# B-R-P/NMSLIB-ZIG

Measured on AMD Instinct MI355X. Metric: queries/sec @ recall@10, 1M x 128-D L2, batch=1024; HBM GB/s vs peak, higher is better.
Workload: dtype f16+f32

## Files before the change

nmslib_zig_amd/csrc/kernels/bf_kernels.hip:

```cpp
#include <cstdio>
#include <type_traits>
#include <vector>
#include <cstdlib>

#include "common_dev.hpp"
#include "kernels.hpp"

namespace gfxknn {

enum BfMode : int { BF_L2 = 0, BF_DOT = 1, BF_COS = 2, BF_L1 = 3, BF_LINF = 4, BF_COSC = 5, BF_L2D = 6 };

struct BfArgs {
    const float* base;
    const float* aux;
    const float* qaux;
    int aux_stride;
    const float* queries;
    u64* cand;
    int* cand_cnt;
    uint32_t* gthr;
    uint32_t* gq;
    int xj, xm;
    int n, ldb, nqt, nsplit, rows_per_split, kprime, cap;
    int kcs;
// ... 1893 lines not shown

__device__ __forceinline__ float one_product_error(const float* qs, int dim, int lane, float bscale, float bres, float scale) {
    float ss = 0.f, rr = 0.f;
    bool over = false;
    for (int d = lane; d < dim; d += 64) {
        const float v = scale * qs[d], w = v - (float)(_Float16)v;
        over |= !(fabsf(v) <= 65504.f);
        ss = fmaf(v, v, ss);
        rr = fmaf(w, w, rr);
    }
    const float qn = sqrtf(wave_sum(ss)), qr = sqrtf(wave_sum(rr));
    if (__any(over)) return INFINITY;
    return 1.01f * (qr * bscale + 1.004f * qn * bres) + 2e-5f * qn * bscale;
}

template <int NPER>
__global__ __launch_bounds__(256) void bf_f32_threshold_kernel(const float* top8, int nlists, int depth, int r, int rcap, int nq,
                                                               int qpad, const float* queries_sel, int ldb, int dim, float bscale,
                                                               float bres, int group_q, int force_precise, float* thr3,
                                                               float* thr1, int* precise, float scale_q, float unit) {
    const int lane = threadIdx.x & 63, q = blockIdx.x * 4 + (threadIdx.x >> 6);
    if (q >= qpad) return;
    if (q >= nq) {
        if (lane == 0) {
            thr3[q] = INFINITY;
            thr1[q] = INFINITY;
        }
        return;
    }
    const int total = nlists * depth;
    uint32_t key[NPER];
#pragma unroll
    for (int i = 0; i < NPER; ++i) {
        const int idx = i * 64 + lane;
        const int l = depth == 4 ? idx >> 2 : idx >> 3, j = idx - l * depth;
        key[i] = idx < total ? f32_ord(top8[((size_t)q * nlists + l) * 8 + j]) : 0u;
    }
    const float e1 = one_product_error(queries_sel + (size_t)q * ldb, dim, lane, bscale, bres, scale_q);
    const uint32_t T = total >= r ? wave_rth_largest_u32<NPER>(key, r) : 0u;
    const float t3 = total >= r ? ord_f32(T) : -INFINITY;
    float t1 = t3;
    bool ok = force_precise != 1;
    if (ok && t3 > -INFINITY) {
        const float need = 2.1f * e1;
        uint32_t best = 0u;
#pragma unroll
        for (int i = 0; i < NPER; ++i) {
            const float v = ord_f32(key[i]);
            const bool c = key[i] != 0u && key[i] <= T && v > -INFINITY && t3 - v >= need;
            best = c && key[i] > best ? key[i] : best;
        }
#pragma unroll
        for (int o = 32; o > 0; o >>= 1) {
// ... 4 lines not shown
        if (best != 0u) {
            int above = 0;
#pragma unroll
            for (int i = 0; i < NPER; ++i) above += __popcll(__builtin_amdgcn_ballot_w64(key[i] > best));
            const int jmax = rcap < total ? rcap : total;
            const int j = best == T ? r : above + 1;
            if (j <= jmax) {
                t1 = ord_f32(best);
                ok = true;
            }
        }
    }
    if (lane == 0) {
        thr3[q] = (t3 - 1.02f * e1) / unit;
        thr1[q] = force_precise == 2 ? INFINITY : t1;
        if (!ok) atomicOr(&precise[q / group_q], 1);
    }
}

struct RerankListF32Args {
    const float* base;
    const float* queries;
    const uint32_t* list;
    const int* list_cnt;
    const int32_t* ext_ids;
    int32_t* out_ids;
    float* out_dists;
    int32_t* out_cnt;
    int* tile_fail;
    int n, k, nsplit, caph, p2max, fail_queries, space, dim, ldb;
    int tps;
    const float* queries_sel;
    const float* thr;
    const float* thr1;
    const int* precise;
    int no_split;
    float bmax;
    float bres;
    float scale, scale_q, bres16;
    int sel_dim, sel_ld;
    const float* qaux;
    unsigned long long* prof;
};

__global__ __launch_bounds__(256) void bf_rerank_f32_list_kernel(RerankListF32Args a) {
    const unsigned long long t0 = a.prof ? wall_clock64() : 0;
    auto lap = [&](int i) __attribute__((always_inline)) {
        if (a.prof && threadIdx.x == 0) atomicAdd(&a.prof[i], wall_clock64() - t0);
    };
    extern __shared__ __attribute__((aligned(16))) char smem[];
    u64* keys = reinterpret_cast<u64*>(smem);
    int* offs = reinterpret_cast<int*>(keys + a.p2max);
    __shared__ int s_over, s_split;
    __shared__ float s_qn2, s_e1, s_thr;
    const int q = blockIdx.x, tid = threadIdx.x, lane = tid & 63, wave = tid >> 6;
    const int nl = 2 * a.nsplit;
    if (tid == 0) s_over = 0;
    __syncthreads();
    if (tid < 64) {
        const int per = (nl + 63) / 64;
        int sum = 0, over = 0;
        for (int i = 0; i < per; ++i) {
            const int s = tid * per + i;
            if (s < nl) {
                const int c = a.list_cnt[(size_t)q * nl + s];
                over |= c > a.caph;
                sum += c < a.caph ? c : a.caph;
            }
        }
        int incl = sum;
#pragma unroll
        for (int o = 1; o < 64; o <<= 1) {
            const int v = __shfl_up(incl, o, 64);
            if (tid >= o) incl += v;
        }
        int run = incl - sum;
        for (int i = 0; i < per; ++i) {
            const int s = tid * per + i;
            if (s < nl) {
                offs[s] = run;
                const int c = a.list_cnt[(size_t)q * nl + s];
                run += c < a.caph ? c : a.caph;
            }
        }
        if (tid == 63) offs[nl] = incl;
        if (__any(over != 0) && tid == 0) s_over = 1;
    } else if (wave == 1) {
        const bool split_product = a.precise[q / a.fail_queries] != 0;
        const float* qs = a.queries_sel + (size_t)q * a.sel_ld;
        float ss = 0.f;
        for (int d = lane; d < a.sel_dim; d += 64) ss = fmaf(qs[d], qs[d], ss);
        ss = wave_sum(ss);
        const float e1 = split_product ? 0.f : one_product_error(qs, a.sel_dim, lane, a.scale * (a.space == SP_L2 || a.space == SP_NEGDOT || a.qaux ? a.bmax : 1.0f), a.bres16, a.scale_q);
        if (lane == 0) {
            s_qn2 = ss;
            s_e1 = e1;
            s_split = split_product ? 1 : 0;
            s_thr = split_product ? a.thr[q] : a.thr1[q];
        }
    }
    __syncthreads();
    const int total = offs[nl];
    if ((a.no_split && a.precise[q / a.fail_queries] != 0) ||
        (a.qaux && a.qaux[(size_t)q * 4 + 3] == 0.f)) {
        if (tid == 0) atomicOr(&a.tile_fail[q / a.fail_queries], 1);
        return;
    }
    const int need = a.k < a.n ? a.k : a.n;
    const int want = need + (a.k / 8 > 4 ? a.k / 8 : 4) < a.n ? need + (a.k / 8 > 4 ? a.k / 8 : 4) : a.n;
    if (s_over || total < want || total > a.p2max) {
        if (tid == 0) atomicOr(&a.tile_fail[q / a.fail_queries], 1);
        return;
    }
    lap(0);
    scan_gather_entries(keys, offs, a.list, q, nl, a.caph, a.tps, tid, blockDim.x);
    __syncthreads();
    lap(1);
    const int P = next_pow2(total < 2 ? 2 : total);
    if (a.prof && tid == 0) {
        atomicAdd(&a.prof[8], (unsigned long long)total);
        atomicAdd(&a.prof[9], (unsigned long long)P);
        atomicAdd(&a.prof[10], 1ull);
    }
    const float* qq = a.queries + (size_t)q * a.ldb;
    const int sub = lane & 15, rg = lane >> 4;
    if (a.dim <= 128) {
        float qv[8];
        bool ok[8];
    #pragma unroll
        for (int c = 0; c < 8; ++c) {
            const int d = sub + 16 * c;
            ok[c] = d < a.dim;
            qv[c] = ok[c] ? qq[d] : 0.f;
        }
        constexpr int kU = 4;
        for (int j0 = wave * (4 * kU); j0 < total; j0 += 16 * kU) {
            uint32_t pos[kU];
            float xv[kU][8];
    #pragma unroll
            for (int u = 0; u < kU; ++u) {
                const int j = j0 + 4 * u + rg;
                pos[u] = (uint32_t)keys[j < total ? j : total - 1];
                const float* row = a.base + (size_t)pos[u] * a.ldb + sub;
    #pragma unroll
                for (int c = 0; c < 8; ++c) xv[u][c] = ok[c] ? row[16 * c] : 0.f;
            }
            __builtin_amdgcn_wave_barrier();
    #pragma unroll
            for (int u = 0; u < kU; ++u) {
                float p0[4], p1[4], p2[4];
    #pragma unroll
                for (int v = 0; v < 4; ++v) {
                    p0[v] = p1[v] = p2[v] = 0.f;
    #pragma unroll
                    for (int c = 0; c < 2; ++c) {
                        if (64 * c >= a.dim) continue;
                        const float x = xv[u][v + 4 * c], y = qv[v + 4 * c];
                        if (a.space == SP_L2) {
                            const float t = x - y;
                            p0[v] = fmaf(t, t, p0[v]);
                        } else {
                            p0[v] = fmaf(x, y, p0[v]);
                            if (a.space != SP_NEGDOT) {
                                p1[v] = fmaf(x, x, p1[v]);
                                p2[v] = fmaf(y, y, p2[v]);
                            }
                        }
                    }
                }
                auto tree = [&](const float* p) __attribute__((always_inline)) -> float {
                    float s = (p[0] + p[2]) + (p[1] + p[3]);
    #pragma unroll
                    for (int o = 8; o > 0; o >>= 1) s += __shfl_xor(s, o, 64);
                    return s;
                };
                const float s0 = tree(p0);
                float d;
                if (a.space == SP_L2) d = sqrtf(s0);
                else if (a.space == SP_NEGDOT) d = -s0;
                else {
                    const float sim = normdot_finish(s0, tree(p1), tree(p2));
                    d = a.space == SP_ANGULAR ? acosf(sim) : fmaxf(0.0f, 1.0f - sim);
                }
                const int j = j0 + 4 * u + rg;
                if (sub == 0 && j < total) keys[j] = ((u64)f32_ord(d) << 32) | pos[u];
            }
        }
    } else {
        const int nstep = (a.dim + 63) >> 6;
        for (int j0 = wave * 16; j0 < total; j0 += 64) {
            uint32_t pos[4];
            const float* rowp[4];
    #pragma unroll
            for (int u = 0; u < 4; ++u) {
                const int j = j0 + 4 * u + rg;
                pos[u] = (uint32_t)keys[j < total ? j : total - 1];
                rowp[u] = a.base + (size_t)pos[u] * a.ldb + sub;
            }
            float p0[4][4], p1[4][4], p2[4][4];
    #pragma unroll
            for (int u = 0; u < 4; ++u)
    #pragma unroll
                for (int v = 0; v < 4; ++v) p0[u][v] = p1[u][v] = p2[u][v] = 0.f;
            for (int c0 = 0; c0 < nstep; c0 += 2) {
                float xv[4][8], qv[8];
                bool ok[8];
    #pragma unroll
                for (int c = 0; c < 8; ++c) {
                    const int d = sub + 16 * (c & 3) + 64 * (c0 + (c >> 2));
                    ok[c] = d < a.dim;
                    qv[c] = ok[c] ? qq[d] : 0.f;
    #pragma unroll
                    for (int u = 0; u < 4; ++u) xv[u][c] = ok[c] ? rowp[u][16 * (c & 3) + 64 * (c0 + (c >> 2))] : 0.f;
                }
    #pragma unroll
                for (int u = 0; u < 4; ++u) {
    #pragma unroll
                    for (int v = 0; v < 4; ++v) {
    #pragma unroll
                        for (int c = 0; c < 2; ++c) {
                            if (64 * (c0 + c) >= a.dim) continue;
                            const float x = xv[u][v + 4 * c], y = qv[v + 4 * c];
                            if (a.space == SP_L2) {
                                const float t = x - y;
                                p0[u][v] = fmaf(t, t, p0[u][v]);
                            } else {
                                p0[u][v] = fmaf(x, y, p0[u][v]);
                                if (a.space != SP_NEGDOT) {
                                    p1[u][v] = fmaf(x, x, p1[u][v]);
                                    p2[u][v] = fmaf(y, y, p2[u][v]);
                                }
                            }
                        }
                    }
                }
            }
            __builtin_amdgcn_wave_barrier();
    #pragma unroll
            for (int u = 0; u < 4; ++u) {
                auto tree = [&](const float* p) __attribute__((always_inline)) -> float {
                    float s = (p[0] + p[2]) + (p[1] + p[3]);
    #pragma unroll
                    for (int o = 8; o > 0; o >>= 1) s += __shfl_xor(s, o, 64);
                    return s;
                };
                const float s0 = tree(p0[u]);
                float d;
                if (a.space == SP_L2) d = sqrtf(s0);
                else if (a.space == SP_NEGDOT) d = -s0;
                else {
                    const float sim = normdot_finish(s0, tree(p1[u]), tree(p2[u]));
                    d = a.space == SP_ANGULAR ? acosf(sim) : fmaxf(0.0f, 1.0f - sim);
                }
                const int j = j0 + 4 * u + rg;
                if (sub == 0 && j < total) keys[j] = ((u64)f32_ord(d) << 32) | pos[u];
            }
        }
    }
    __syncthreads();
    lap(2);
    if (total <= 512 && a.k <= 32) {
        __shared__ u64 s_head[128];
        const int e0 = wave * 128 + 2 * lane;
        u64 k0 = e0 < total ? keys[e0] : ~0ull, k1 = e0 + 1 < total ? keys[e0 + 1] : ~0ull;
        wave_sort128_u64(k0, k1, lane);
        if (lane < 16) {
            s_head[wave * 32 + 2 * lane] = k0;
            s_head[wave * 32 + 2 * lane + 1] = k1;
        }
        __syncthreads();
        if (wave == 0) {
            k0 = s_head[2 * lane];
            k1 = s_head[2 * lane + 1];
            wave_sort128_u64(k0, k1, lane);
            if (lane < 16) {
                keys[2 * lane] = k0;
                keys[2 * lane + 1] = k1;
            }
        }
        __syncthreads();
    } else {
        for (int i = total + tid; i < P; i += blockDim.x) keys[i] = ~0ull;
        __syncthreads();
        block_bitonic_u64_asc(keys, P, tid, blockDim.x);
    }
    lap(3);
    const int found = total < a.k ? total : a.k;
    if (total < a.n) {
        const bool split_product = s_split != 0;
        if (tid == 0) {
            const float qn2 = s_qn2, qn = sqrtf(qn2);
            const float dk = ord_f32((uint32_t)(keys[found - 1] >> 32));
            float sk, e, extra = 0.f;
            if (a.qaux) {
                const float sh = sinf(0.5f * dk);
                const float omc = a.space == SP_ANGULAR ? 2.0f * sh * sh : dk;
                const float qnorm = a.qaux[(size_t)q * 4 + 2];
                sk = -omc * qnorm;
                e = 6.1036e-5f * qn * a.bmax;
                extra = 1e-6f * qn * a.bmax + 2e-6f * qnorm;
            } else if (a.space == SP_L2) {
                sk = 0.5f * (qn2 - dk * dk);
                e = 6.1036e-5f * qn * a.bmax;
            } else if (a.space == SP_NEGDOT) {
                sk = -dk;
                e = 6.1036e-5f * qn * a.bmax;
            } else {
                sk = (a.space == SP_ANGULAR ? cosf(dk) : 1.0f - dk) * qn;
                e = 6.1036e-5f * qn;
            }
            const float t = s_thr;
            if (!split_product) {
                const float unit = a.scale * a.scale_q;
                sk *= unit;
                extra *= unit;
                e = s_e1;
            }
            e += extra + 1e-6f * (fabsf(sk) + fabsf(t));
            if (!(sk - t >= e)) atomicOr(&a.tile_fail[q / a.fail_queries], 1);
        }
    }
    lap(4);
    for (int i = tid; i < a.k; i += blockDim.x) {
        int32_t id = -1;
        float d = INFINITY;
        if (i < found) {
            const u64 key = keys[i];
            const uint32_t pos = (uint32_t)key;
            id = a.ext_ids ? a.ext_ids[pos] : (int32_t)pos;
            d = ord_f32((uint32_t)(key >> 32));
        }
        a.out_ids[(size_t)q * a.k + i] = id;
        a.out_dists[(size_t)q * a.k + i] = d;
    }
    if (tid == 0 && a.out_cnt) a.out_cnt[q] = found;
    lap(5);
}

__global__ void row_maxnorm_kernel(const float* rows, int n, int ld, int dim, int relative, unsigned* out_bits, float scale16) {
    const int lane = threadIdx.x & 63;
    const int wpb = blockDim.x >> 6;
    float mb = 0.f, mr = 0.f, ma = 0.f, mh = 0.f;
    for (int row = blockIdx.x * wpb + (threadIdx.x >> 6); row < n; row += gridDim.x * wpb) {
        const float* p = rows + (size_t)row * ld;
        float s = 0.f, r = 0.f, rh = 0.f;
        for (int d = lane; d < dim; d += 64) {
            const float v = p[d], w = v - (float)(__bf16)v;
            const float vs = scale16 * v, wh = vs - (float)(_Float16)vs;
            s = fmaf(v, v, s);
            r = fmaf(w, w, r);
            rh = fmaf(wh, wh, rh);
// ... 21 lines not shown
    const void* queries;
    const u64* cand;
    const int* cand_cnt;
    const int32_t* ext_ids;
    int32_t* out_ids;
    float* out_dists;
    int32_t* out_cnt;
    int space, dim, ldb, k, nsplit, cap, kprime, p2max;
    const int* tile_fail;
    int fail_queries;
    int* verify_flags;
    int verify_queries;
    const float* queries_sel;
    float bmax;
    float eps_rel;
};

__global__ __launch_bounds__(256) void bf_rerank_kernel(RerankArgs a) {
    extern __shared__ __attribute__((aligned(16))) char smem[];
    u64* keys = reinterpret_cast<u64*>(smem);
    int* offs = reinterpret_cast<int*>(keys + a.p2max);
    const int q = blockIdx.x, tid = threadIdx.x, lane = tid & 63, wave = tid >> 6;
    if (a.tile_fail && a.tile_fail[q / a.fail_queries] == 0) return;

    if (tid == 0) {
        int o = 0;
        for (int s = 0; s < a.nsplit; ++s) {
            offs[s] = o;
            int c = a.cand_cnt[(size_t)q * a.nsplit + s];
            o += c < a.kprime ? c : a.kprime;
        }
        offs[a.nsplit] = o;
    }
    __syncthreads();
    const int total = offs[a.nsplit];
    __shared__ uint32_t s_kth;
    const bool verify = a.verify_flags != nullptr && a.space == SP_L2 && total >= a.kprime;
    if (tid == 0) s_kth = 0xffffffffu;
// ... 76 lines not shown
            const float* qs = a.queries_sel + (size_t)q * a.ldb;
            float ss = 0.f;
            for (int d = tid; d < a.dim; d += 64) ss = fmaf(qs[d], qs[d], ss);
            ss = wave_sum(ss);
            if (tid == 0) s_qn2v = ss;
        }
        __syncthreads();
        if (tid == 0) {
            const float qn2 = s_qn2v, qn = sqrtf(qn2);
            const float kth = ord_f32(s_kth);
            const float dk = ord_f32((uint32_t)(keys[found - 1] >> 32));
            const float e = a.eps_rel * (qn * a.bmax + 0.5f * a.bmax * a.bmax);
            const float floor_d2 = qn2 - 2.0f * kth - 2.0f * e - 2e-6f * (qn2 + fabsf(kth));
            if (!(dk * dk <= floor_d2)) atomicOr(&a.verify_flags[q / a.verify_queries], 1);
        }
    }
}

__global__ void row_aux_f32_kernel(const float* base, int n, int ldb, int dim, int space, float* aux) {
    const int lane = threadIdx.x & 63;
    const int row = blockIdx.x * (blockDim.x >> 6) + (threadIdx.x >> 6);
    if (row >= n) return;
    const float* p = base + (size_t)row * ldb;
    float s = 0.f;
    for (int d = lane; d < dim; d += 64) s = fmaf(p[d], p[d], s);
    s = wave_sum(s);
    if (lane == 0) {
        float v = 0.f;
        if (space == SP_L2) v = -0.5f * s;
        else if (space == SP_COSINE || space == SP_ANGULAR)
// ... 522 lines not shown
                            const int* cand_cnt, const int32_t* ext_ids, int32_t* out_ids,
                            float* out_dists, int32_t* out_cnt, hipStream_t s) {
    return launch_bf_rerank_ex(p, space, dim, k, base, queries_padded, cand, cand_cnt, ext_ids, out_ids, out_dists,
                               out_cnt, nullptr, 1, s);
}

hipError_t launch_bf_rerank_ex(const BfPlan& p, int space, int dim, int k, const void* base,
                               const void* queries_padded, const unsigned long long* cand,
                               const int* cand_cnt, const int32_t* ext_ids, int32_t* out_ids,
                               float* out_dists, int32_t* out_cnt, const int* tile_fail, int fail_queries,
                               hipStream_t s) {
    return launch_bf_rerank_verify(p, space, dim, k, base, queries_padded, cand, cand_cnt, ext_ids, out_ids, out_dists,
                                   out_cnt, tile_fail, fail_queries, nullptr, nullptr, 0.f, s);
}

hipError_t launch_bf_rerank_verify(const BfPlan& p, int space, int dim, int k, const void* base,
                                   const void* queries_padded, const unsigned long long* cand,
                                   const int* cand_cnt, const int32_t* ext_ids, int32_t* out_ids,
                                   float* out_dists, int32_t* out_cnt, const int* tile_fail, int fail_queries,
                                   int* verify_flags, const float* queries_sel, float bmax, hipStream_t s) {
    RerankArgs a{};
    a.verify_flags = verify_flags;
    a.verify_queries = BF_TQ;
    a.queries_sel = queries_sel;
    a.bmax = bmax;
    a.eps_rel = 1.5f * (float)(dim + 2) * 5.9604645e-8f;
    a.tile_fail = tile_fail;
    a.fail_queries = fail_queries;
    a.base = base;
    a.queries = queries_padded;
// ... 2 lines not shown
    a.ext_ids = ext_ids;
    a.out_ids = out_ids;
    a.out_dists = out_dists;
    a.out_cnt = out_cnt;
    a.space = space;
    a.dim = dim;
    a.ldb = p.ldb;
    a.k = k;
    a.nsplit = p.nsplit;
    a.cap = p.cap;
    a.kprime = p.kprime;
    a.p2max = p.p2max;
    hipError_t e = hipFuncSetAttribute(reinterpret_cast<const void*>(bf_rerank_kernel),
                                       hipFuncAttributeMaxDynamicSharedMemorySize, (int)p.lds_rerank);
    if (e != hipSuccess) return e;
    hipLaunchKernelGGL(bf_rerank_kernel, dim3(p.nq), dim3(256), p.lds_rerank, s, a);
    return hipGetLastError();
}

hipError_t launch_bf_adaptive_f32(const BfPlan& p, int space, int dim, int k, const float* base_orig, const float* sel_rows,
                                  const float* aux, const float* queries_orig, const float* queries_sel,
                                  const float* qaux_cosc, float bmax, unsigned long long* cand, int* cand_cnt, int* flags,
                                  const int32_t* ext_ids, int32_t* out_ids, float* out_dists, int32_t* out_cnt,
                                  const int* gate, int gate_tiles, hipStream_t s, bool cleared) {
    hipError_t e = launch_bf_select_f32_ex(p, space, sel_rows, aux, queries_sel, qaux_cosc, cand, cand_cnt, gate, gate_tiles, s,
                                           cleared);
    if (e != hipSuccess) return e;
    const bool verify = space == SP_L2 && flags != nullptr && bmax > 0.f;
    if (!verify)
        return launch_bf_rerank_ex(p, space, dim, k, base_orig, queries_orig, cand, cand_cnt, ext_ids, out_ids, out_dists,
                                   out_cnt, gate, gate_tiles * BF_TQ, s);
// ... 180 lines not shown
    if (const char* e = getenv("NMSLIB_GPU_SAMPLE_STRIDE")) f.stride = atoi(e) > 0 ? atoi(e) : 16;
    const int kp = k + (k / 8 > 4 ? k / 8 : 4);
    const double kf = (double)kp / f.stride;
    f.r = (int)(1.6 * kf + 3.0 * sqrt(kf) + 3.0 + 0.999);
    f.rcap = 4 * f.r + 32;
    f.force_precise = false;
    if (const char* e = getenv("NMSLIB_GPU_F32_TERMS")) f.force_precise = atoi(e) == 3;
    const int tiles_all = (n + BF_BN - 1) / BF_BN;
    int ns = (256 + f.nqt - 1) / f.nqt;
    if (ns > tiles_all / 16) ns = tiles_all / 16;
    if (ns > 256) ns = 256;
    ns = (ns + 7) / 8 * 8;
    if (ns < 8) ns = 8;
    while ((tiles_all + ns - 1) / ns > 32768) ns += 8;
    f.nsplit = ns;
    f.tps = (tiles_all + ns - 1) / ns;
    const double mean_half = (double)f.rcap * f.stride / (2.0 * ns);
    int caph = 8;
    while (caph < 3.0 * mean_half + 8.0) caph <<= 1;
    f.caph = caph;
    f.p2max = host_next_pow2((int)(2.5 * f.rcap * f.stride) + 64);
    if (f.p2max > 2 * ns * caph) f.p2max = host_next_pow2(2 * ns * caph);
    f.lds_scan = 4 * 2 * BF_BN * 256 + 8 * BF_BN * 4 + 64;
    f.lds_scan1 = 9 * BF_BN * 256 + 16 * BF_BN * 4 + 64;
    f.lds_rerank = (size_t)f.p2max * 8 + (2 * (size_t)ns + 1) * 4 + 16;
    const int stiles = (tiles_all + f.stride - 1) / f.stride;
    const int s_nqt = f.qpad / (f.kch > 1 ? 128 : 256);
    int nss = (256 + s_nqt - 1) / s_nqt;
    if (nss > stiles / 16) nss = stiles / 16;
    if (nss > 64) nss = 64;
// ... 76 lines not shown
    if (qg == 2) return launch_scan_f32_one<MODE, false, 4>(a, grid, lds, s);
    return launch_scan_f32_one<MODE, false, 2>(a, grid, lds, s);
}

hipError_t launch_bf_f32_fast(const BfF32Fast& f, int space, int n, int dim, int ldb, int nq, int k, const float* base_orig,
                              const float* sel_rows, const float* aux, const void* base_hi, const void* base_lo,
                              const float* auxp, float bmax, float bres, const float* queries_orig, const float* queries_sel,
                              void* q_hi, void* q_lo, float* top8, unsigned long long* cand_fb, int* cnt_fb, float* thr,
                              uint32_t* list, int* list_cnt, int* tile_fail, int* flags_fb, const int32_t* ext_ids,
                              int32_t* out_ids, float* out_dists, int32_t* out_cnt, hipEvent_t scan_begin,
                              hipEvent_t scan_end, hipStream_t s, const float* queries_raw, float* queries_pad_out,
                              const float* qaux_cosc, const float* queries_centred, int sel_ld, const BfF16Side& h16) {
    const int sdim = f.cosc ? f.sel_dim : dim, sld = f.cosc ? sel_ld : ldb;
    float* thr1 = thr + f.qpad;
    int* precise = tile_fail + f.nqt;
    hipError_t e;
    {
        const BfPlan& fb = f.fallback;
        uint32_t* gthr = reinterpret_cast<uint32_t*>(cnt_fb + (size_t)fb.qpad * fb.nsplit);
        const size_t gwords = 2 * ((size_t)fb.qpad + (size_t)fb.qpad * fb.nsplit);
        size_t work = (size_t)f.qpad * f.dp > gwords ? (size_t)f.qpad * f.dp : gwords;
        size_t grid = (work + 255) / 256;
        if (grid > 2048) grid = 2048;
        hipLaunchKernelGGL(bf_f32_prep_kernel, dim3((unsigned)grid), dim3(256), 0, s, queries_raw, nq, sdim, queries_sel, f.qpad,
                           sld, queries_pad_out, f.kch > 1 ? nullptr : static_cast<__bf16*>(q_hi),
                           f.kch > 1 ? nullptr : static_cast<__bf16*>(q_lo),
                           tile_fail, 2 * f.nqt, flags_fb, fb.nqt, gthr, gwords, f.dp, static_cast<_Float16*>(h16.q_h16), h16.scale_q);
        e = hipGetLastError();
        if (e != hipSuccess) return e;
    }
// ... 20 lines not shown
    a.nqt = f.nqt;
    BfScanF32Args sa = a;
    sa.nqt = f.qpad / (f.kch > 1 ? 128 : 256);
    sa.nsplit = f.s_nsplit;
    sa.tps = f.s_tps;
    sa.tile_stride = f.stride;
    sa.top8 = top8;
    e = scan(sa, true, 1, 8 * sa.nqt * (f.s_nsplit / 8));
    if (e != hipSuccess) return e;
    {
        static const bool dbg_nohit = getenv("NMSLIB_GPU_DEBUG") && (atoi(getenv("NMSLIB_GPU_DEBUG")) & 8192);
        const int depth = f.rcap <= 64 && f.s_nsplit >= 32 ? 4 : 8;
        const dim3 tgrid((f.qpad + 3) / 4);
#define BF_THR_ARGS                                                                                                               \
    top8, 2 * f.s_nsplit, depth, f.r, f.rcap, nq, f.qpad, queries_sel, sld, sdim, h16.scale * (f.mode == 2 ? 1.0f : bmax), h16.bres16, f.tq, \
        f.force_precise ? 1 : (dbg_nohit ? 2 : 0), thr, thr1, precise, h16.scale_q, h16.scale * h16.scale_q
        if (2 * f.s_nsplit * depth <= 512) hipLaunchKernelGGL(bf_f32_threshold_kernel<8>, tgrid, dim3(256), 0, s, BF_THR_ARGS);
        else hipLaunchKernelGGL(bf_f32_threshold_kernel<16>, tgrid, dim3(256), 0, s, BF_THR_ARGS);
#undef BF_THR_ARGS
    }
    e = hipGetLastError();
    if (e != hipSuccess) return e;
    a.list = list;
    a.list_cnt = list_cnt;
    a.nsplit = f.nsplit;
    a.tps = f.tps;
    a.caph = f.caph;
    a.tile_stride = 1;
    a.group_flag = precise;
    const int grid = 8 * f.nqt * (f.nsplit / 8);
    if (scan_begin) (void)hipEventRecord(scan_begin, s);
// ... 26 lines not shown
    r.p2max = f.p2max;
    r.fail_queries = f.tq;
    r.no_split = f.kch > 1 ? 1 : 0;
    r.space = space;
    r.dim = dim;
    r.ldb = ldb;
    r.queries_sel = queries_sel;
    r.sel_dim = sdim;
    r.sel_ld = sld;
    r.scale = h16.scale;
    r.scale_q = h16.scale_q;
    r.bres16 = h16.bres16;
    r.qaux = f.cosc ? qaux_cosc : nullptr;
    r.thr = thr;
    r.thr1 = thr1;
    r.precise = precise;
    r.bmax = bmax;
    r.bres = bres;
    static const int dbg_prof = getenv("NMSLIB_GPU_DEBUG") ? atoi(getenv("NMSLIB_GPU_DEBUG")) : 0;
    static unsigned long long* d_prof = nullptr;
    if (dbg_prof & 4096) {
        if (!d_prof) (void)hipMalloc(&d_prof, 16 * 8);
        (void)hipMemsetAsync(d_prof, 0, 16 * 8, s);
        r.prof = d_prof;
    }
    e = hipFuncSetAttribute(reinterpret_cast<const void*>(bf_rerank_f32_list_kernel),
                            hipFuncAttributeMaxDynamicSharedMemorySize, (int)f.lds_rerank);
    if (e != hipSuccess) return e;
    hipLaunchKernelGGL(bf_rerank_f32_list_kernel, dim3(nq), dim3(256), f.lds_rerank, s, r);
    e = hipGetLastError();
    if (e != hipSuccess) return e;
    if (dbg_prof & 4096) {
        unsigned long long h[16];
        (void)hipStreamSynchronize(s);
        (void)hipMemcpy(h, d_prof, sizeof(h), hipMemcpyDeviceToHost);
        const double wg = h[10] ? (double)h[10] : 1.0;
        fprintf(stderr, "[rerank f32 list] workgroups %llu rows/query %.1f P %.1f | us since start: prefix %.2f gather %.2f distances %.2f "
                "sort %.2f proof %.2f out %.2f\n", h[10], h[8] / wg, h[9] / wg, h[0] / wg / 100, h[1] / wg / 100, h[2] / wg / 100,
                h[3] / wg / 100, h[4] / wg / 100, h[5] / wg / 100);
    }
    {
        static const int dbg = getenv("NMSLIB_GPU_DEBUG") ? atoi(getenv("NMSLIB_GPU_DEBUG")) : 0;
        if (dbg & 2048) {
            (void)hipStreamSynchronize(s);
// ... 134 lines not shown
```

nmslib_zig_amd/csrc/kernels/kernels.hpp:

```cpp
#pragma once
#include <hip/hip_runtime_api.h>
#include <stddef.h>
#include <stdint.h>

namespace gfxknn {

enum SpaceCode : int {
    SP_L2 = 0,
    SP_L1 = 1,
    SP_LINF = 2,
    SP_COSINE = 3,
    SP_ANGULAR = 4,
    SP_NEGDOT = 5,
    SP_L2SQR_SIFT = 6,
    SP_L2SQR = 7,
    SP_NORMCOS = 8,
    SP_QNORM_NEGDOT = 9,
    SP_LEVEN = 10,
    SP_BIT_HAMMING = 11,
};

constexpr int BF_TQ = 128;
constexpr int BF_BN = 64;
constexpr int BF_KC = 128;
// ... 74 lines not shown
    bool cosc;
    int sel_dim;
    int kch;
    int dp;
    int tq;
    int qpad, nqt;
    int stride, r;
    int rcap;
    bool force_precise;
    int nsplit, tps, caph, p2max;
    int s_nsplit, s_tps;
    size_t lds_scan, lds_scan1, lds_thr, lds_rerank;
    BfPlan fallback;
};
BfF32Fast bf_f32_fast_plan(int n, int dim, int nq, int k, int space, bool cosine_centred);
inline size_t bf_f32_thr_bytes(const BfF32Fast& f) { return (size_t)f.qpad * 8 + (size_t)f.nqt * 8 + 64; }
inline size_t bf_f32_list_elems(const BfF32Fast& f) { return (size_t)f.qpad * f.nsplit * 2 * f.caph; }
inline size_t bf_f32_listcnt_elems(const BfF32Fast& f) { return (size_t)f.qpad * f.nsplit * 2; }
inline size_t bf_f32_top8_elems(const BfF32Fast& f) { return (size_t)f.qpad * f.s_nsplit * 2 * 8; }
inline int bf_f32_rows_padded(int n) { return (n + BF_BN - 1) / BF_BN * BF_BN + BF_BN; }
hipError_t launch_row_maxnorm(const float* rows, int n, int ld, int dim, bool relative_residual, float* out, hipStream_t s,
                              float scale16 = 0.f);
hipError_t launch_split_bf16(const float* src, int rows, int rows_pad, int ld, int dim, void* hi, void* lo,
                             const float* aux, float aux_pad, float* auxp, hipStream_t s, int dp = 128, void* h16 = nullptr,
                             float scale = 1.f, float* auxp16 = nullptr, float aux16_mul = 1.f);
struct BfF16Side {
    const void* base_h16;
    const float* auxp16;
    void* q_h16;
    float scale;
    float bres16;
// ... 247 lines not shown
```

Baseline: 2.911 million.

## Make rerank kernels persistent with prefetched list headers and hoisted query norms

The f32 list rerank kernel becomes persistent: each workgroup loops over several queries and prefetches the next query's list counts and first entries while processing the current one. The prefix scan moves from a single wave to the whole block. Gather expansion is done inline per thread instead of through a separate helper. Row and query loads are vectorised to float4 with a new 16-lane tree reduction, and the query norm and one-product error are computed once in the threshold kernel and passed through a buffer. The verify rerank kernel also gets a grid-stride loop capped at the CU count. The aim is to cut launch and tail costs, redundant per-query norm work and scalar loads, at the cost of extra registers, an enlarged threshold buffer, and new alignment preconditions that make unaligned inputs return an error.

```diff
diff --git a/nmslib_zig_amd/csrc/kernels/bf_kernels.hip b/nmslib_zig_amd/csrc/kernels/bf_kernels.hip
--- a/nmslib_zig_amd/csrc/kernels/bf_kernels.hip
+++ b/nmslib_zig_amd/csrc/kernels/bf_kernels.hip
@@ -1931,11 +1931,18 @@
     return 1.01f * (qr * bscale + 1.004f * qn * bres) + 2e-5f * qn * bscale;
 }
 
+__device__ __forceinline__ float query_norm2(const float* qs, int dim, int lane) {
+    float ss = 0.f;
+    for (int d = lane; d < dim; d += 64) ss = fmaf(qs[d], qs[d], ss);
+    return wave_sum(ss);
+}
+
 template <int NPER>
 __global__ __launch_bounds__(256) void bf_f32_threshold_kernel(const float* top8, int nlists, int depth, int r, int rcap, int nq,
                                                                int qpad, const float* queries_sel, int ldb, int dim, float bscale,
                                                                float bres, int group_q, int force_precise, float* thr3,
-                                                               float* thr1, int* precise, float scale_q, float unit) {
+                                                               float* thr1, int* precise, float scale_q, float unit,
+                                                               float* qe1, float* qn2) {
     const int lane = threadIdx.x & 63, q = blockIdx.x * 4 + (threadIdx.x >> 6);
     if (q >= qpad) return;
     if (q >= nq) {
@@ -1954,6 +1961,7 @@
         key[i] = idx < total ? f32_ord(top8[((size_t)q * nlists + l) * 8 + j]) : 0u;
     }
     const float e1 = one_product_error(queries_sel + (size_t)q * ldb, dim, lane, bscale, bres, scale_q);
+    const float n2 = query_norm2(queries_sel + (size_t)q * ldb, dim, lane);
     const uint32_t T = total >= r ? wave_rth_largest_u32<NPER>(key, r) : 0u;
     const float t3 = total >= r ? ord_f32(T) : -INFINITY;
     float t1 = t3;
@@ -1988,6 +1996,8 @@
     if (lane == 0) {
         thr3[q] = (t3 - 1.02f * e1) / unit;
         thr1[q] = force_precise == 2 ? INFINITY : t1;
+        qe1[q] = e1;
+        qn2[q] = n2;
         if (!ok) atomicOr(&precise[q / group_q], 1);
     }
 }
@@ -2014,301 +2024,310 @@
     float scale, scale_q, bres16;
     int sel_dim, sel_ld;
     const float* qaux;
+    const float* qe1;
+    const float* qn2;
+    int nq;
     unsigned long long* prof;
 };
 
+__device__ __forceinline__ float row16_tree_sum(const float* p, int sub) {
+    const bool hi8 = (sub & 8) != 0, hi4 = (sub & 4) != 0;
+    float k0 = hi8 ? p[2] : p[0], k1 = hi8 ? p[3] : p[1];
+    const float g0 = hi8 ? p[0] : p[2], g1 = hi8 ? p[1] : p[3];
+    k0 += __shfl_xor(g0, 8, 64);
+    k1 += __shfl_xor(g1, 8, 64);
+    float t = hi4 ? k1 : k0;
+    t += __shfl_xor(hi4 ? k0 : k1, 4, 64);
+    t += __shfl_xor(t, 2, 64);
+    t += __shfl_xor(t, 1, 64);
+    t += __shfl_xor(t, 8, 64);
+    t += __shfl_xor(t, 4, 64);
+    return t;
+}
+
 __global__ __launch_bounds__(256) void bf_rerank_f32_list_kernel(RerankListF32Args a) {
-    const unsigned long long t0 = a.prof ? wall_clock64() : 0;
-    auto lap = [&](int i) __attribute__((always_inline)) {
-        if (a.prof && threadIdx.x == 0) atomicAdd(&a.prof[i], wall_clock64() - t0);
-    };
     extern __shared__ __attribute__((aligned(16))) char smem[];
     u64* keys = reinterpret_cast<u64*>(smem);
-    int* offs = reinterpret_cast<int*>(keys + a.p2max);
-    __shared__ int s_over, s_split;
-    __shared__ float s_qn2, s_e1, s_thr;
-    const int q = blockIdx.x, tid = threadIdx.x, lane = tid & 63, wave = tid >> 6;
+    __shared__ int s_wsum[4];
+    __shared__ u64 s_head[128];
+    const int tid = threadIdx.x, lane = tid & 63, wave = tid >> 6;
     const int nl = 2 * a.nsplit;
-    if (tid == 0) s_over = 0;
-    __syncthreads();
-    if (tid < 64) {
-        const int per = (nl + 63) / 64;
-        int sum = 0, over = 0;
-        for (int i = 0; i < per; ++i) {
-            const int s = tid * per + i;
-            if (s < nl) {
-                const int c = a.list_cnt[(size_t)q * nl + s];
-                over |= c > a.caph;
-                sum += c < a.caph ? c : a.caph;
-            }
+    const int lpt = (nl + 255) >> 8;
+    struct Lists {
+        int cnt[2];
+        uint32_t ent[2][2];
+    };
+    auto request = [&](Lists& L, int q) __attribute__((always_inline)) {
+#pragma unroll
+        for (int i = 0; i < 2; ++i) {
+            const int s = tid * lpt + i;
+            const bool have = i < lpt && s < nl;
+            const uint32_t* e = a.list + (size_t)q * a.caph * nl + s;
+            L.cnt[i] = have ? a.list_cnt[(size_t)q * nl + s] : 0;
+            L.ent[i][0] = have ? e[0] : 0u;
+            L.ent[i][1] = have ? e[nl] : 0u;
+        }
+    };
+    Lists cur = {}, nxt = {};
+    if ((int)blockIdx.x < a.nq) request(cur, blockIdx.x);
+    for (int q = blockIdx.x; q < a.nq; q += gridDim.x, cur = nxt) {
+        const unsigned long long t0 = a.prof ? wall_clock64() : 0;
+        auto lap = [&](int i) __attribute__((always_inline)) {
+            if (a.prof && tid == 0) atomicAdd(&a.prof[i], wall_clock64() - t0);
+        };
+        __syncthreads();
+        if (q + (int)gridDim.x < a.nq) request(nxt, q + gridDim.x);
+        const bool split_product = a.precise[q / a.fail_queries] != 0;
+        float pr_thr = 0.f, pr_e1 = 0.f, pr_qn2 = 0.f;
+        if (tid == 0) {
+            pr_thr = split_product ? a.thr[q] : a.thr1[q];
+            pr_e1 = a.qe1[q];
+            pr_qn2 = a.qn2[q];
+        }
+        int cl[2], sum = 0;
+        bool over = false;
+#pragma unroll
+        for (int i = 0; i < 2; ++i) {
+            over |= cur.cnt[i] > a.caph;
+            cl[i] = cur.cnt[i] < a.caph ? cur.cnt[i] : a.caph;
+            sum += cl[i];
         }
         int incl = sum;
 #pragma unroll
         for (int o = 1; o < 64; o <<= 1) {
             const int v = __shfl_up(incl, o, 64);
-            if (tid >= o) incl += v;
-        }
+            if (lane >= o) incl += v;
+        }
+        if (lane == 63) s_wsum[wave] = incl;
+        const int any_over = __syncthreads_or(over ? 1 : 0);
         int run = incl - sum;
-        for (int i = 0; i < per; ++i) {
-            const int s = tid * per + i;
-            if (s < nl) {
-                offs[s] = run;
-                const int c = a.list_cnt[(size_t)q * nl + s];
-                run += c < a.caph ? c : a.caph;
-            }
-        }
-        if (tid == 63) offs[nl] = incl;
-        if (__any(over != 0) && tid == 0) s_over = 1;
-    } else if (wave == 1) {
-        const bool split_product = a.precise[q / a.fail_queries] != 0;
-        const float* qs = a.queries_sel + (size_t)q * a.sel_ld;
-        float ss = 0.f;
-        for (int d = lane; d < a.sel_dim; d += 64) ss = fmaf(qs[d], qs[d], ss);
-        ss = wave_sum(ss);
-        const float e1 = split_product ? 0.f : one_product_error(qs, a.sel_dim, lane, a.scale * (a.space == SP_L2 || a.space == SP_NEGDOT || a.qaux ? a.bmax : 1.0f), a.bres16, a.scale_q);
-        if (lane == 0) {
-            s_qn2 = ss;
-            s_e1 = e1;
-            s_split = split_product ? 1 : 0;
-            s_thr = split_product ? a.thr[q] : a.thr1[q];
-        }
-    }
-    __syncthreads();
-    const int total = offs[nl];
-    if ((a.no_split && a.precise[q / a.fail_queries] != 0) ||
-        (a.qaux && a.qaux[(size_t)q * 4 + 3] == 0.f)) {
-        if (tid == 0) atomicOr(&a.tile_fail[q / a.fail_queries], 1);
-        return;
-    }
-    const int need = a.k < a.n ? a.k : a.n;
-    const int want = need + (a.k / 8 > 4 ? a.k / 8 : 4) < a.n ? need + (a.k / 8 > 4 ? a.k / 8 : 4) : a.n;
-    if (s_over || total < want || total > a.p2max) {
-        if (tid == 0) atomicOr(&a.tile_fail[q / a.fail_queries], 1);
-        return;
-    }
-    lap(0);
-    scan_gather_entries(keys, offs, a.list, q, nl, a.caph, a.tps, tid, blockDim.x);
-    __syncthreads();
-    lap(1);
-    const int P = next_pow2(total < 2 ? 2 : total);
-    if (a.prof && tid == 0) {
-        atomicAdd(&a.prof[8], (unsigned long long)total);
-        atomicAdd(&a.prof[9], (unsigned long long)P);
-        atomicAdd(&a.prof[10], 1ull);
-    }
-    const float* qq = a.queries + (size_t)q * a.ldb;
-    const int sub = lane & 15, rg = lane >> 4;
-    if (a.dim <= 128) {
-        float qv[8];
-        bool ok[8];
-    #pragma unroll
-        for (int c = 0; c < 8; ++c) {
-            const int d = sub + 16 * c;
-            ok[c] = d < a.dim;
-            qv[c] = ok[c] ? qq[d] : 0.f;
-        }
-        constexpr int kU = 4;
-        for (int j0 = wave * (4 * kU); j0 < total; j0 += 16 * kU) {
-            uint32_t pos[kU];
-            float xv[kU][8];
-    #pragma unroll
-            for (int u = 0; u < kU; ++u) {
-                const int j = j0 + 4 * u + rg;
-                pos[u] = (uint32_t)keys[j < total ? j : total - 1];
-                const float* row = a.base + (size_t)pos[u] * a.ldb + sub;
-    #pragma unroll
-                for (int c = 0; c < 8; ++c) xv[u][c] = ok[c] ? row[16 * c] : 0.f;
-            }
-            __builtin_amdgcn_wave_barrier();
-    #pragma unroll
-            for (int u = 0; u < kU; ++u) {
-                float p0[4], p1[4], p2[4];
-    #pragma unroll
-                for (int v = 0; v < 4; ++v) {
-                    p0[v] = p1[v] = p2[v] = 0.f;
-    #pragma unroll
-                    for (int c = 0; c < 2; ++c) {
-                        if (64 * c >= a.dim) continue;
-                        const float x = xv[u][v + 4 * c], y = qv[v + 4 * c];
-                        if (a.space == SP_L2) {
-                            const float t = x - y;
-                            p0[v] = fmaf(t, t, p0[v]);
-                        } else {
-                            p0[v] = fmaf(x, y, p0[v]);
-                            if (a.space != SP_NEGDOT) {
-                                p1[v] = fmaf(x, x, p1[v]);
-                                p2[v] = fmaf(y, y, p2[v]);
-                            }
-                        }
+#pragma unroll
+        for (int w = 0; w < 4; ++w) run += w < wave ? s_wsum[w] : 0;
+        const int total = s_wsum[0] + s_wsum[1] + s_wsum[2] + s_wsum[3];
+        if ((a.no_split && split_product) ||
+            (a.qaux && a.qaux[(size_t)q * 4 + 3] == 0.f)) {
+            if (tid == 0) atomicOr(&a.tile_fail[q / a.fail_queries], 1);
+            continue;
+        }
+        const int need = a.k < a.n ? a.k : a.n;
+        const int want = need + (a.k / 8 > 4 ? a.k / 8 : 4) < a.n ? need + (a.k / 8 > 4 ? a.k / 8 : 4) : a.n;
+        if (any_over || total < want || total > a.p2max) {
+            if (tid == 0) atomicOr(&a.tile_fail[q / a.fail_queries], 1);
+            continue;
+        }
+        lap(0);
+#pragma unroll
+        for (int i = 0; i < 2; ++i) {
+            const int len = cl[i];
+            if (len == 0) continue;
+            const int s = tid * lpt + i;
+            const uint32_t* e = a.list + (size_t)q * a.caph * nl + s;
+            const uint32_t row_base = (uint32_t)(s >> 1) * (uint32_t)a.tps * BF_BN + 4u * (s & 1);
+            int j = 0;
+            auto expand = [&](const uint32_t ent) __attribute__((always_inline)) {
+                uint32_t m = ent & 0xffffu;
+                const uint32_t r0 = row_base + (ent >> 16) * 32u;
+                while (m && j < len) {
+                    const int bit = 31 - __builtin_clz(m);
+                    m &= ~(1u << bit);
+                    const int reg = 15 - bit;
+                    keys[run + j++] = (u64)(r0 + (reg & 3) + 8 * (reg >> 2));
+                }
+            };
+            expand(cur.ent[i][0]);
+            if (j < len) expand(cur.ent[i][1]);
+            for (int i0 = 2; i0 < a.caph && j < len; i0 += 4) {
+                uint32_t pre[4];
+#pragma unroll
+                for (int t = 0; t < 4; ++t) pre[t] = (i0 + t < len && i0 + t < a.caph) ? e[(size_t)(i0 + t) * nl] : 0u;
+#pragma unroll
+                for (int t = 0; t < 4; ++t)
+                    if (i0 + t < a.caph && j < len) expand(pre[t]);
+            }
+            run += len;
+        }
+        __syncthreads();
+        lap(1);
+        const int P = next_pow2(total < 2 ? 2 : total);
+        if (a.prof && tid == 0) {
+            atomicAdd(&a.prof[8], (unsigned long long)total);
+            atomicAdd(&a.prof[9], (unsigned long long)P);
+            atomicAdd(&a.prof[10], 1ull);
+        }
+        typedef float f32x4 __attribute__((ext_vector_type(4)));
+        const float* qq = a.queries + (size_t)q * a.ldb;
+        const int sub = lane & 15, rg = lane >> 4;
+        const f32x4 zero4 = {0.f, 0.f, 0.f, 0.f};
+        auto fetch = [&](const float* row, int st) __attribute__((always_inline)) -> f32x4 {
+            const int d0 = 64 * st + 4 * sub;
+            f32x4 v = d0 < a.dim ? *reinterpret_cast<const f32x4*>(row + d0) : zero4;
+#pragma unroll
+            for (int i = 0; i < 4; ++i) v[i] = d0 + i < a.dim ? v[i] : 0.f;
+            return v;
+        };
+        auto chain = [&](float* p0, float* p1, float* p2, const f32x4 x, const f32x4 y) __attribute__((always_inline)) {
+#pragma unroll
+            for (int v = 0; v < 4; ++v) {
+                if (a.space == SP_L2) {
+                    const float t = x[v] - y[v];
+                    p0[v] = fmaf(t, t, p0[v]);
+                } else {
+                    p0[v] = fmaf(x[v], y[v], p0[v]);
+                    if (a.space != SP_NEGDOT) {
+                        p1[v] = fmaf(x[v], x[v], p1[v]);
+                        p2[v] = fmaf(y[v], y[v], p2[v]);
                     }
                 }
-                auto tree = [&](const float* p) __attribute__((always_inline)) -> float {
-                    float s = (p[0] + p[2]) + (p[1] + p[3]);
-    #pragma unroll
-                    for (int o = 8; o > 0; o >>= 1) s += __shfl_xor(s, o, 64);
-                    return s;
-                };
-                const float s0 = tree(p0);
-                float d;
-                if (a.space == SP_L2) d = sqrtf(s0);
-                else if (a.space == SP_NEGDOT) d = -s0;
-                else {
-                    const float sim = normdot_finish(s0, tree(p1), tree(p2));
-                    d = a.space == SP_ANGULAR ? acosf(sim) : fmaxf(0.0f, 1.0f - sim);
+            }
+        };
+        auto finish = [&](const float* p0, const float* p1, const float* p2) __attribute__((always_inline)) -> float {
+            const float s0 = row16_tree_sum(p0, sub);
+            if (a.space == SP_L2) return sqrtf(s0);
+            if (a.space == SP_NEGDOT) return -s0;
+            const float sim = normdot_finish(s0, row16_tree_sum(p1, sub), row16_tree_sum(p2, sub));
+            return a.space == SP_ANGULAR ? acosf(sim) : fmaxf(0.0f, 1.0f - sim);
+        };
+        if (a.dim <= 128) {
+            const f32x4 qv0 = fetch(qq, 0), qv1 = fetch(qq, 1);
+            constexpr int kU = 4;
+            for (int j0 = wave * (4 * kU); j0 < total; j0 += 16 * kU) {
+                uint32_t pos[kU];
+                f32x4 xv[kU][2];
+#pragma unroll
+                for (int u = 0; u < kU; ++u) {
+                    const int j = j0 + 4 * u + rg;
+                    pos[u] = (uint32_t)keys[j < total ? j : total - 1];
+                    const float* row = a.base + (size_t)pos[u] * a.ldb;
+                    xv[u][0] = fetch(row, 0);
+                    xv[u][1] = fetch(row, 1);
                 }
-                const int j = j0 + 4 * u + rg;
-                if (sub == 0 && j < total) keys[j] = ((u64)f32_ord(d) << 32) | pos[u];
-            }
-        }
-    } else {
-        const int nstep = (a.dim + 63) >> 6;
-        for (int j0 = wave * 16; j0 < total; j0 += 64) {
-            uint32_t pos[4];
-            const float* rowp[4];
-    #pragma unroll
-            for (int u = 0; u < 4; ++u) {
-                const int j = j0 + 4 * u + rg;
-                pos[u] = (uint32_t)keys[j < total ? j : total - 1];
-                rowp[u] = a.base + (size_t)pos[u] * a.ldb + sub;
-            }
-            float p0[4][4], p1[4][4], p2[4][4];
-    #pragma unroll
-            for (int u = 0; u < 4; ++u)
-    #pragma unroll
-                for (int v = 0; v < 4; ++v) p0[u][v] = p1[u][v] = p2[u][v] = 0.f;
-            for (int c0 = 0; c0 < nstep; c0 += 2) {
-                float xv[4][8], qv[8];
-                bool ok[8];
-    #pragma unroll
-                for (int c = 0; c < 8; ++c) {
-                    const int d = sub + 16 * (c & 3) + 64 * (c0 + (c >> 2));
-                    ok[c] = d < a.dim;
-                    qv[c] = ok[c] ? qq[d] : 0.f;
-    #pragma unroll
-                    for (int u = 0; u < 4; ++u) xv[u][c] = ok[c] ? rowp[u][16 * (c & 3) + 64 * (c0 + (c >> 2))] : 0.f;
+                __builtin_amdgcn_wave_barrier();
+#pragma unroll
+                for (int u = 0; u < kU; ++u) {
+                    float p0[4] = {0.f, 0.f, 0.f, 0.f}, p1[4] = {0.f, 0.f, 0.f, 0.f}, p2[4] = {0.f, 0.f, 0.f, 0.f};
+                    chain(p0, p1, p2, xv[u][0], qv0);
+                    if (a.dim > 64) chain(p0, p1, p2, xv[u][1], qv1);
+                    const float d = finish(p0, p1, p2);
+                    const int j = j0 + 4 * u + rg;
+                    if (sub == 0 && j < total) keys[j] = ((u64)f32_ord(d) << 32) | pos[u];
                 }
-    #pragma unroll
+            }
+        } else {
+            const int nstep = (a.dim + 63) >> 6;
+            for (int j0 = wave * 16; j0 < total; j0 += 64) {
+                uint32_t pos[4];
+                const float* rowp[4];
+#pragma unroll
                 for (int u = 0; u < 4; ++u) {
-    #pragma unroll
-                    for (int v = 0; v < 4; ++v) {
-    #pragma unroll
-                        for (int c = 0; c < 2; ++c) {
-                            if (64 * (c0 + c) >= a.dim) continue;
-                            const float x = xv[u][v + 4 * c], y = qv[v + 4 * c];
-                            if (a.space == SP_L2) {
-                                const float t = x - y;
-                                p0[u][v] = fmaf(t, t, p0[u][v]);
-                            } else {
-                                p0[u][v] = fmaf(x, y, p0[u][v]);
-                                if (a.space != SP_NEGDOT) {
-                                    p1[u][v] = fmaf(x, x, p1[u][v]);
-                                    p2[u][v] = fmaf(y, y, p2[u][v]);
-                                }
-                            }
-                        }
+                    const int j = j0 + 4 * u + rg;
+                    pos[u] = (uint32_t)keys[j < total ? j : total - 1];
+                    rowp[u] = a.base + (size_t)pos[u] * a.ldb;
+                }
+                float p0[4][4], p1[4][4], p2[4][4];
+#pragma unroll
+                for (int u = 0; u < 4; ++u)
+#pragma unroll
+                    for (int v = 0; v < 4; ++v) p0[u][v] = p1[u][v] = p2[u][v] = 0.f;
+                for (int c0 = 0; c0 < nstep; c0 += 2) {
+                    f32x4 xv[4][2];
+                    const f32x4 qv0 = fetch(qq, c0), qv1 = fetch(qq, c0 + 1);
+#pragma unroll
+                    for (int u = 0; u < 4; ++u) {
+                        xv[u][0] = fetch(rowp[u], c0);
+                        xv[u][1] = fetch(rowp[u], c0 + 1);
+                    }
+#pragma unroll
+                    for (int u = 0; u < 4; ++u) {
+                        chain(p0[u], p1[u], p2[u], xv[u][0], qv0);
+                        if (64 * (c0 + 1) < a.dim) chain(p0[u], p1[u], p2[u], xv[u][1], qv1);
                     }
                 }
-            }
-            __builtin_amdgcn_wave_barrier();
-    #pragma unroll
-            for (int u = 0; u < 4; ++u) {
-                auto tree = [&](const float* p) __attribute__((always_inline)) -> float {
-                    float s = (p[0] + p[2]) + (p[1] + p[3]);
-    #pragma unroll
-                    for (int o = 8; o > 0; o >>= 1) s += __shfl_xor(s, o, 64);
-                    return s;
-                };
-                const float s0 = tree(p0[u]);
-                float d;
-                if (a.space == SP_L2) d = sqrtf(s0);
-                else if (a.space == SP_NEGDOT) d = -s0;
-                else {
-                    const float sim = normdot_finish(s0, tree(p1[u]), tree(p2[u]));
-                    d = a.space == SP_ANGULAR ? acosf(sim) : fmaxf(0.0f, 1.0f - sim);
+                __builtin_amdgcn_wave_barrier();
+#pragma unroll
+                for (int u = 0; u < 4; ++u) {
+                    const float d = finish(p0[u], p1[u], p2[u]);
+                    const int j = j0 + 4 * u + rg;
+                    if (sub == 0 && j < total) keys[j] = ((u64)f32_ord(d) << 32) | pos[u];
                 }
-                const int j = j0 + 4 * u + rg;
-                if (sub == 0 && j < total) keys[j] = ((u64)f32_ord(d) << 32) | pos[u];
-            }
-        }
-    }
-    __syncthreads();
-    lap(2);
-    if (total <= 512 && a.k <= 32) {
-        __shared__ u64 s_head[128];
-        const int e0 = wave * 128 + 2 * lane;
-        u64 k0 = e0 < total ? keys[e0] : ~0ull, k1 = e0 + 1 < total ? keys[e0 + 1] : ~0ull;
-        wave_sort128_u64(k0, k1, lane);
-        if (lane < 16) {
-            s_head[wave * 32 + 2 * lane] = k0;
-            s_head[wave * 32 + 2 * lane + 1] = k1;
+            }
         }
         __syncthreads();
-        if (wave == 0) {
-            k0 = s_head[2 * lane];
-            k1 = s_head[2 * lane + 1];
+        lap(2);
+        if (total <= 512 && a.k <= 32) {
+            const int e0 = wave * 128 + 2 * lane;
+            u64 k0 = e0 < total ? keys[e0] : ~0ull, k1 = e0 + 1 < total ? keys[e0 + 1] : ~0ull;
             wave_sort128_u64(k0, k1, lane);
             if (lane < 16) {
-                keys[2 * lane] = k0;
-                keys[2 * lane + 1] = k1;
-            }
-        }
-        __syncthreads();
-    } else {
-        for (int i = total + tid; i < P; i += blockDim.x) keys[i] = ~0ull;
-        __syncthreads();
-        block_bitonic_u64_asc(keys, P, tid, blockDim.x);
-    }
-    lap(3);
-    const int found = total < a.k ? total : a.k;
-    if (total < a.n) {
-        const bool split_product = s_split != 0;
-        if (tid == 0) {
-            const float qn2 = s_qn2, qn = sqrtf(qn2);
-            const float dk = ord_f32((uint32_t)(keys[found - 1] >> 32));
-            float sk, e, extra = 0.f;
-            if (a.qaux) {
-                const float sh = sinf(0.5f * dk);
-                const float omc = a.space == SP_ANGULAR ? 2.0f * sh * sh : dk;
-                const float qnorm = a.qaux[(size_t)q * 4 + 2];
-                sk = -omc * qnorm;
-                e = 6.1036e-5f * qn * a.bmax;
-                extra = 1e-6f * qn * a.bmax + 2e-6f * qnorm;
-            } else if (a.space == SP_L2) {
-                sk = 0.5f * (qn2 - dk * dk);
-                e = 6.1036e-5f * qn * a.bmax;
-            } else if (a.space == SP_NEGDOT) {
-                sk = -dk;
-                e = 6.1036e-5f * qn * a.bmax;
-            } else {
-                sk = (a.space == SP_ANGULAR ? cosf(dk) : 1.0f - dk) * qn;
-                e = 6.1036e-5f * qn;
-            }
-            const float t = s_thr;
-            if (!split_product) {
-                const float unit = a.scale * a.scale_q;
-                sk *= unit;
-                extra *= unit;
-                e = s_e1;
-            }
-            e += extra + 1e-6f * (fabsf(sk) + fabsf(t));
-            if (!(sk - t >= e)) atomicOr(&a.tile_fail[q / a.fail_queries], 1);
-        }
-    }
-    lap(4);
-    for (int i = tid; i < a.k; i += blockDim.x) {
-        int32_t id = -1;
-        float d = INFINITY;
-        if (i < found) {
-            const u64 key = keys[i];
-            const uint32_t pos = (uint32_t)key;
-            id = a.ext_ids ? a.ext_ids[pos] : (int32_t)pos;
-            d = ord_f32((uint32_t)(key >> 32));
-        }
-        a.out_ids[(size_t)q * a.k + i] = id;
-        a.out_dists[(size_t)q * a.k + i] = d;
-    }
-    if (tid == 0 && a.out_cnt) a.out_cnt[q] = found;
-    lap(5);
+                s_head[wave * 32 + 2 * lane] = k0;
+                s_head[wave * 32 + 2 * lane + 1] = k1;
+            }
+            __syncthreads();
+            if (wave == 0) {
+                k0 = s_head[2 * lane];
+                k1 = s_head[2 * lane + 1];
+                wave_sort128_u64(k0, k1, lane);
+                if (lane < 16) {
+                    keys[2 * lane] = k0;
+                    keys[2 * lane + 1] = k1;
+                }
+            }
+            __syncthreads();
+        } else {
+            for (int i = total + tid; i < P; i += blockDim.x) keys[i] = ~0ull;
+            __syncthreads();
+            block_bitonic_u64_asc(keys, P, tid, blockDim.x);
+        }
+        lap(3);
+        const int found = total < a.k ? total : a.k;
+        if (total < a.n) {
+            if (tid == 0) {
+                const float qn2 = pr_qn2, qn = sqrtf(qn2);
+                const float dk = ord_f32((uint32_t)(keys[found - 1] >> 32));
+                float sk, e, extra = 0.f;
+                if (a.qaux) {
+                    const float sh = sinf(0.5f * dk);
+                    const float omc = a.space == SP_ANGULAR ? 2.0f * sh * sh : dk;
+                    const float qnorm = a.qaux[(size_t)q * 4 + 2];
+                    sk = -omc * qnorm;
+                    e = 6.1036e-5f * qn * a.bmax;
+                    extra = 1e-6f * qn * a.bmax + 2e-6f * qnorm;
+                } else if (a.space == SP_L2) {
+                    sk = 0.5f * (qn2 - dk * dk);
+                    e = 6.1036e-5f * qn * a.bmax;
+                } else if (a.space == SP_NEGDOT) {
+                    sk = -dk;
+                    e = 6.1036e-5f * qn * a.bmax;
+                } else {
+                    sk = (a.space == SP_ANGULAR ? cosf(dk) : 1.0f - dk) * qn;
+                    e = 6.1036e-5f * qn;
+                }
+                const float t = pr_thr;
+                if (!split_product) {
+                    const float unit = a.scale * a.scale_q;
+                    sk *= unit;
+                    extra *= unit;
+                    e = pr_e1;
+                }
+                e += extra + 1e-6f * (fabsf(sk) + fabsf(t));
+                if (!(sk - t >= e)) atomicOr(&a.tile_fail[q / a.fail_queries], 1);
+            }
+        }
+        lap(4);
+        for (int i = tid; i < a.k; i += blockDim.x) {
+            int32_t id = -1;
+            float d = INFINITY;
+            if (i < found) {
+                const u64 key = keys[i];
+                const uint32_t pos = (uint32_t)key;
+                id = a.ext_ids ? a.ext_ids[pos] : (int32_t)pos;
+                d = ord_f32((uint32_t)(key >> 32));
+            }
+            a.out_ids[(size_t)q * a.k + i] = id;
+            a.out_dists[(size_t)q * a.k + i] = d;
+        }
+        if (tid == 0 && a.out_cnt) a.out_cnt[q] = found;
+        lap(5);
+    }
 }
 
 __global__ void row_maxnorm_kernel(const float* rows, int n, int ld, int dim, int relative, unsigned* out_bits, float scale16) {
@@ -2360,14 +2379,13 @@
     const float* queries_sel;
     float bmax;
     float eps_rel;
+    int nq;
 };
 
-__global__ __launch_bounds__(256) void bf_rerank_kernel(RerankArgs a) {
-    extern __shared__ __attribute__((aligned(16))) char smem[];
+__device__ __forceinline__ void bf_rerank_query(const RerankArgs& a, const int q, char* smem) {
     u64* keys = reinterpret_cast<u64*>(smem);
     int* offs = reinterpret_cast<int*>(keys + a.p2max);
-    const int q = blockIdx.x, tid = threadIdx.x, lane = tid & 63, wave = tid >> 6;
-    if (a.tile_fail && a.tile_fail[q / a.fail_queries] == 0) return;
+    const int tid = threadIdx.x, lane = tid & 63, wave = tid >> 6;
 
     if (tid == 0) {
         int o = 0;
@@ -2474,6 +2492,15 @@
             const float floor_d2 = qn2 - 2.0f * kth - 2.0f * e - 2e-6f * (qn2 + fabsf(kth));
             if (!(dk * dk <= floor_d2)) atomicOr(&a.verify_flags[q / a.verify_queries], 1);
         }
+    }
+}
+
+__global__ __launch_bounds__(256) void bf_rerank_kernel(RerankArgs a) {
+    extern __shared__ __attribute__((aligned(16))) char smem[];
+    for (int q = blockIdx.x; q < a.nq; q += gridDim.x) {
+        if (a.tile_fail && a.tile_fail[q / a.fail_queries] == 0) continue;
+        bf_rerank_query(a, q, smem);
+        __syncthreads();
     }
 }
 
@@ -3026,6 +3053,15 @@
                                    out_cnt, tile_fail, fail_queries, nullptr, nullptr, 0.f, s);
 }
 
+static int device_cu_count() {
+    static const int cus = [] {
+        int dev = 0, n = 0;
+        if (hipGetDevice(&dev) != hipSuccess || hipDeviceGetAttribute(&n, hipDeviceAttributeMultiprocessorCount, dev) != hipSuccess) n = 0;
+        return n > 0 ? n : 256;
+    }();
+    return cus;
+}
+
 hipError_t launch_bf_rerank_verify(const BfPlan& p, int space, int dim, int k, const void* base,
                                    const void* queries_padded, const unsigned long long* cand,
                                    const int* cand_cnt, const int32_t* ext_ids, int32_t* out_ids,
@@ -3058,7 +3094,15 @@
     hipError_t e = hipFuncSetAttribute(reinterpret_cast<const void*>(bf_rerank_kernel),
                                        hipFuncAttributeMaxDynamicSharedMemorySize, (int)p.lds_rerank);
     if (e != hipSuccess) return e;
-    hipLaunchKernelGGL(bf_rerank_kernel, dim3(p.nq), dim3(256), p.lds_rerank, s, a);
+    a.nq = p.nq;
+    int grid = p.nq;
+    if (tile_fail) {
+        const int cap = device_cu_count();
+        static const int cap_env = getenv("NMSLIB_GPU_TAIL_GRID") ? atoi(getenv("NMSLIB_GPU_TAIL_GRID")) : 0;
+        const int c = cap_env > 0 ? cap_env : cap;
+        if (grid > c) grid = c;
+    }
+    hipLaunchKernelGGL(bf_rerank_kernel, dim3(grid), dim3(256), p.lds_rerank, s, a);
     return hipGetLastError();
 }
 
@@ -3269,6 +3313,10 @@
     if (ns < 8) ns = 8;
     while ((tiles_all + ns - 1) / ns > 32768) ns += 8;
     f.nsplit = ns;
+    if (2 * ns > 512) {
+        f.use = false;
+        return f;
+    }
     f.tps = (tiles_all + ns - 1) / ns;
     const double mean_half = (double)f.rcap * f.stride / (2.0 * ns);
     int caph = 8;
@@ -3375,6 +3423,10 @@
     const int sdim = f.cosc ? f.sel_dim : dim, sld = f.cosc ? sel_ld : ldb;
     float* thr1 = thr + f.qpad;
     int* precise = tile_fail + f.nqt;
+    float* qe1 = reinterpret_cast<float*>(precise + f.nqt);
+    float* qn2 = qe1 + f.qpad;
+    if (ldb % 4 != 0 || (reinterpret_cast<uintptr_t>(base_orig) | reinterpret_cast<uintptr_t>(queries_orig)) % 16 != 0)
+        return hipErrorInvalidValue;
     hipError_t e;
     {
         const BfPlan& fb = f.fallback;
@@ -3425,7 +3477,7 @@
         const dim3 tgrid((f.qpad + 3) / 4);
 #define BF_THR_ARGS                                                                                                               \
     top8, 2 * f.s_nsplit, depth, f.r, f.rcap, nq, f.qpad, queries_sel, sld, sdim, h16.scale * (f.mode == 2 ? 1.0f : bmax), h16.bres16, f.tq, \
-        f.force_precise ? 1 : (dbg_nohit ? 2 : 0), thr, thr1, precise, h16.scale_q, h16.scale * h16.scale_q
+        f.force_precise ? 1 : (dbg_nohit ? 2 : 0), thr, thr1, precise, h16.scale_q, h16.scale * h16.scale_q, qe1, qn2
         if (2 * f.s_nsplit * depth <= 512) hipLaunchKernelGGL(bf_f32_threshold_kernel<8>, tgrid, dim3(256), 0, s, BF_THR_ARGS);
         else hipLaunchKernelGGL(bf_f32_threshold_kernel<16>, tgrid, dim3(256), 0, s, BF_THR_ARGS);
 #undef BF_THR_ARGS
@@ -3482,6 +3534,9 @@
     r.qaux = f.cosc ? qaux_cosc : nullptr;
     r.thr = thr;
     r.thr1 = thr1;
+    r.qe1 = qe1;
+    r.qn2 = qn2;
+    r.nq = nq;
     r.precise = precise;
     r.bmax = bmax;
     r.bres = bres;
@@ -3495,7 +3550,11 @@
     e = hipFuncSetAttribute(reinterpret_cast<const void*>(bf_rerank_f32_list_kernel),
                             hipFuncAttributeMaxDynamicSharedMemorySize, (int)f.lds_rerank);
     if (e != hipSuccess) return e;
-    hipLaunchKernelGGL(bf_rerank_f32_list_kernel, dim3(nq), dim3(256), f.lds_rerank, s, r);
+    const int cus = device_cu_count();
+    static const int qpw_env = getenv("NMSLIB_GPU_RERANK_QPW") ? atoi(getenv("NMSLIB_GPU_RERANK_QPW")) : 0;
+    const int resident = 4 * cus;
+    const int qpw = qpw_env > 0 ? qpw_env : (nq + resident - 1) / resident;
+    hipLaunchKernelGGL(bf_rerank_f32_list_kernel, dim3((nq + qpw - 1) / qpw), dim3(256), f.lds_rerank, s, r);
     e = hipGetLastError();
     if (e != hipSuccess) return e;
     if (dbg_prof & 4096) {
diff --git a/nmslib_zig_amd/csrc/kernels/kernels.hpp b/nmslib_zig_amd/csrc/kernels/kernels.hpp
--- a/nmslib_zig_amd/csrc/kernels/kernels.hpp
+++ b/nmslib_zig_amd/csrc/kernels/kernels.hpp
@@ -112,7 +112,7 @@
     BfPlan fallback;
 };
 BfF32Fast bf_f32_fast_plan(int n, int dim, int nq, int k, int space, bool cosine_centred);
-inline size_t bf_f32_thr_bytes(const BfF32Fast& f) { return (size_t)f.qpad * 8 + (size_t)f.nqt * 8 + 64; }
+inline size_t bf_f32_thr_bytes(const BfF32Fast& f) { return (size_t)f.qpad * 16 + (size_t)f.nqt * 8 + 64; }
 inline size_t bf_f32_list_elems(const BfF32Fast& f) { return (size_t)f.qpad * f.nsplit * 2 * f.caph; }
 inline size_t bf_f32_listcnt_elems(const BfF32Fast& f) { return (size_t)f.qpad * f.nsplit * 2; }
 inline size_t bf_f32_top8_elems(const BfF32Fast& f) { return (size_t)f.qpad * f.s_nsplit * 2 * 8; }
```

After: 2.853 million. 0.98x the previous value.
